# ITBE-Lab/ma

Measured on AMD Instinct MI355X. Metric: aligned reads/sec (whole node), 150bp & 10kb synthetic vs GRCh38, higher is better.
Workload: dtype u8/int8 (2-bit BWT ranks, int8 DP differences, int16/32 scores); 1 GPU; 20000000 x 150 bp reads (0.50% sub, 0.00% ins, 0.00% del), default preset, 1000000 reads/step per GPU vs GRCh38-like synthetic genome (24 contigs, 3088269832 nt, planted repeats)

## Files before the change

ma_amd/csrc/launch_seed.h:

```cpp
static SeedParams seed_params( const ma_params& P )
{
    SeedParams S;
    S.technique = (u32)P.seeding_technique;
    S.min_seed_len = (u32)P.min_seed_len;
    S.min_amb = (u32)P.min_ambiguity;
    S.max_amb = (u32)P.max_ambiguity;
    S.min_seed_size_drop = (u32)P.min_seed_size_drop;
    S.disable_heuristics = (u32)P.disable_heuristics;
    S.rel_min_seed_size_amount = P.rel_min_seed_size_amount;
    S.genome_size_disable = P.genome_size_disable;
    S.window_begin = S.window_end = nullptr;
    S.smem_compact = 0;
    S.smem_merge = 0;
    return S;
}
static void seed_window( SeedParams& S, const ma_batch* b, bool on )
{
    const u64 bytes = b->n_bases + ( b->reads_external ? 0 : 64 );
    if( const char* e = getenv( "MA_SEED_WINDOW" ) )
        on = on && atoi( e ) != 0;
    if( on && bytes >= 16 )
    {
        S.window_begin = b->d_reads;
        S.window_end = b->d_reads + bytes;
    }
}

static int seed_mems( ma_batch* b )
{
    const u64 n = b->n_reads, nb = b->n_bases;
    if( b->segOff.reserve( ( n + 1 ) * 8 ) || b->segCnt.reserve( ( n + 1 ) * 4 ) || b->memsCnt.reserve( ( nb + 2 ) * 8 ) ||
        b->memsOff.reserve( ( nb + 2 ) * 8 ) )
        return 1;
    MemsArgs A;
    A.X = b->idx->v;
    A.P = seed_params( b->P );
    A.reads = b->d_reads;
    A.roff = b->d_roff;
    A.n_reads = (u32)n;
    A.n_bases = nb;
    A.cnt = b->memsCnt.as<u64>( );
    A.off = b->memsOff.as<u64>( );
    A.pool = nullptr;
    A.pool_read = nullptr;
    A.ctr = b->ctr.as<unsigned long long>( );
    EvTimer t( b, 0 );
    u64 total = 0;
    if( nb )
    {
        hipLaunchKernelGGL( k_mems<false>, dim3( (unsigned)( ( nb + 255 ) / 256 ) ), dim3( 256 ), 0, b->stream, A );
        MA_HIP( hipMemsetAsync( (char*)b->memsCnt.p + nb * 8, 0, 8, b->stream ) );
        if( scan_exclusive<u64>( b, b->memsCnt.as<u64>( ), b->memsOff.as<u64>( ), nb + 1 ) )
            return 1;
        MA_HIP( hipMemcpyAsync( &total, (char*)b->memsOff.p + nb * 8, 8, hipMemcpyDeviceToHost, b->stream ) );
        if( batch_wait( b ) )
        return 1;
    }
    else
        MA_HIP( hipMemsetAsync( b->memsOff.p, 0, 16, b->stream ) );
    b->segPoolCap = std::max<u64>( total + 1024, b->segPoolCap );
    if( b->segPool.reserve( b->segPoolCap * sizeof( ma_segment ) ) || b->segRead.reserve( b->segPoolCap * 4 ) )
        return 1;
    A.pool = b->segPool.as<ma_segment>( );
    A.pool_read = b->segRead.as<u32>( );
    if( nb && total )
        hipLaunchKernelGGL( k_mems<true>, dim3( (unsigned)( ( nb + 255 ) / 256 ) ), dim3( 256 ), 0, b->stream, A );
    hipLaunchKernelGGL( k_mems_finish, dim3( (unsigned)( ( n + 255 ) / 256 ) ), dim3( 256 ), 0, b->stream, A.X, A.P, b->d_roff, (u32)n,
                        b->memsOff.as<u64>( ), b->segPool.as<ma_segment>( ), b->segOff.as<u64>( ), b->segCnt.as<u32>( ) );
    const unsigned long long used = total;
    MA_HIP( hipMemcpyAsync( b->ctr.as<unsigned long long>( ) + CTR_SEG_USED, &used, 8, hipMemcpyHostToDevice, b->stream ) );
    if( batch_wait( b ) )
        return 1;
    MA_HIP( hipGetLastError( ) );
    return 0;
}

static u64 seg_pool_heuristic( u64 n_bases, u64 n_reads )
{
    return std::max<u64>( n_bases / 16 + 16 * n_reads, 1024 );
}

static int seed_tasks( ma_batch* b )
{
    const u64 n = b->n_reads, nb = b->n_bases;
    int levels = 2;
    for( u32 q = b->max_qlen; q > 1; q >>= 1 )
        levels++;
    if( levels >= MA_TASK_KEY_BITS / 2 )
        return 2;
    const bool smem = b->P.seeding_technique == 1;
    const u64 taskCap = nb / 16 + 2 * n + 1024;
    b->segPoolCap = std::max( ( smem ? 4 : 1 ) * seg_pool_heuristic( nb, n ), b->segPoolMin );
    u32 segCapT = 96, smemCapT = 384;
    if( const char* e = getenv( "MA_SEED_TASK_CAPS" ) )
    {
        int a = 0, c = 0;
        if( sscanf( e, "%d,%d", &a, &c ) == 2 && a > 0 && c > 0 )
            segCapT = (u32)a, smemCapT = (u32)( ( c + 1 ) & ~1 );
    }
    const u32 smem_compact = smem && b->max_qlen < ( 1u << MA_SMEM_QZ_BITS ) && b->idx->v.n < ( 1ull << 35 ) && !( getenv( "MA_SMEM_COMPACT" ) && atoi( getenv( "MA_SMEM_COMPACT" ) ) == 0 ) ? 1 : 0;
    const u64 smemEntry = smem_compact ? 16 : sizeof( ma_segment );
    unsigned blocksT = smem ? 1024 : 2048;
    if( const char* e = getenv( "MA_SEED_TASK_BLOCKS" ) )
        blocksT = (unsigned)std::max( 64, std::min( 4096, atoi( e ) ) );
    const u64 lanesT = (u64)blocksT * 256;
    if( smem && ( b->taskStage.reserve( lanesT * segCapT * sizeof( ma_segment ) ) || b->smemA.reserve( lanesT * smemCapT * smemEntry ) ||
                  b->smemB.reserve( lanesT * smemCapT * smemEntry ) ) )
        return 1;
    if( b->segOff.reserve( ( n + 1 ) * 8 ) || b->segCnt.reserve( ( n + 1 ) * 4 ) || b->taskA.reserve( taskCap * sizeof( SeedTask ) ) ||
        b->taskB.reserve( taskCap * sizeof( SeedTask ) ) || b->taskCnt.reserve( 64 * 8 ) ||
        b->segPool.reserve( b->segPoolCap * sizeof( ma_segment ) ) || b->segRead.reserve( b->segPoolCap * 4 ) ||
        b->stage.reserve( b->segPoolCap * sizeof( ma_segment ) ) || b->taskKey.reserve( b->segPoolCap * 8 ) ||
        b->taskKey2.reserve( b->segPoolCap * 8 ) || b->taskPerm.reserve( b->segPoolCap * 4 ) || b->taskPerm2.reserve( b->segPoolCap * 4 ) )
        return 1;
    unsigned long long* cnt = b->taskCnt.as<unsigned long long>( );
    MA_HIP( hipMemsetAsync( cnt, 0, 64 * 8, b->stream ) );
    TaskKernelArgs A;
    A.X = b->idx->v;
    A.P = seed_params( b->P );
    seed_window( A.P, b, true );
    A.slow_batch = 4;
    if( const char* e = getenv( "MA_SEED_SLOW_BATCH" ) )
        A.slow_batch = (u32)std::max( 1, atoi( e ) );
    A.reads = b->d_reads;
    A.roff = b->d_roff;
    A.task_cap = taskCap;
    A.pool = b->stage.as<ma_segment>( );
    A.pool_key = b->taskKey.as<u64>( );
    A.pool_cap = b->segPoolCap;
    A.ctr = b->ctr.as<unsigned long long>( );
    A.stage = smem ? b->taskStage.as<ma_segment>( ) : nullptr;
    A.seg_cap = segCapT;
    A.smem_a = smem ? b->smemA.as<ma_segment>( ) : nullptr;
    A.smem_b = smem ? b->smemB.as<ma_segment>( ) : nullptr;
    A.smem_cap = smemCapT;
    if( smem )
    {
        A.P.smem_compact = smem_compact;
        A.P.smem_merge = A.P.min_amb == 0 ? 1 : 0;
        if( const char* e = getenv( "MA_SMEM_MERGE" ) )
            A.P.smem_merge = A.P.smem_merge && atoi( e ) != 0 ? 1 : 0;
        A.X.kmer_k = 0;
        A.slow_batch = 8;
        if( const char* e = getenv( "MA_SEED_SLOW_BATCH" ) )
            A.slow_batch = (u32)std::max( 1, atoi( e ) );
    }
    {
        EvTimer t( b, 0 );
        hipLaunchKernelGGL( k_task_roots, dim3( (unsigned)( ( n + 255 ) / 256 ) ), dim3( 256 ), 0, b->stream, b->d_roff, (u32)n,
                            b->taskA.as<SeedTask>( ), cnt );
        for( int lv = 0; lv < levels; lv++ )
        {
            A.in = ( lv & 1 ) ? b->taskB.as<SeedTask>( ) : b->taskA.as<SeedTask>( );
            A.out = ( lv & 1 ) ? b->taskA.as<SeedTask>( ) : b->taskB.as<SeedTask>( );
            A.nIn = cnt + lv;
            A.nOut = cnt + lv + 1;
            MA_HIP( hipMemsetAsync( A.ctr + CTR_NEXT_READ, 0, 8, b->stream ) );
            if( smem )
                hipLaunchKernelGGL( k_seed_tasks_smem, dim3( blocksT ), dim3( 256 ), 0, b->stream, A );
            else
                hipLaunchKernelGGL( k_seed_tasks, dim3( blocksT ), dim3( 256 ), 0, b->stream, A );
        }
    }
    MA_HIP( hipGetLastError( ) );
    if( read_ctr( b ) )
        return 1;
    const u32 err = (u32)b->hctr[ CTR_ERR ];
    const u64 ns = b->hctr[ CTR_SEG_USED ];
    if( ( err & ( MA_ERR_STACK_OVERFLOW | MA_ERR_SMEM_OVERFLOW ) ) )
    {
        MA_HIP( hipMemsetAsync( b->ctr.p, 0, CTR_COUNT * 8, b->stream ) );
        return 2;
    }
    if( ( err & MA_ERR_SEG_OVERFLOW ) || ns > b->segPoolCap )
    {
        b->segPoolMin = ns + 1024;
        MA_HIP( hipMemsetAsync( b->ctr.p, 0, CTR_COUNT * 8, b->stream ) );
        return seed_tasks( b );
    }
    MA_HIP( hipMemsetAsync( b->segCnt.p, 0, ( n + 1 ) * 4, b->stream ) );
    if( ns )
    {
        hipLaunchKernelGGL( k_iota32, dim3( (unsigned)( ( ns + 255 ) / 256 ) ), dim3( 256 ), 0, b->stream, b->taskPerm.as<u32>( ), ns );
        size_t tb = 0;
        MA_HIP( hipcub::DeviceRadixSort::SortPairs( nullptr, tb, b->taskKey.as<u64>( ), b->taskKey2.as<u64>( ), b->taskPerm.as<u32>( ),
                                                    b->taskPerm2.as<u32>( ), (int)ns, 0, 64, b->stream ) );
        if( b->cubTmp.reserve( tb + 256 ) )
            return 1;
        MA_HIP( hipcub::DeviceRadixSort::SortPairs( b->cubTmp.p, tb, b->taskKey.as<u64>( ), b->taskKey2.as<u64>( ), b->taskPerm.as<u32>( ),
                                                    b->taskPerm2.as<u32>( ), (int)ns, 0, 64, b->stream ) );
        const dim3 grid( (unsigned)( ( ns + 255 ) / 256 ) ), block( 256 );
        hipLaunchKernelGGL( k_task_permute, grid, block, 0, b->stream, b->stage.as<ma_segment>( ), b->taskKey2.as<u64>( ),
                            b->taskPerm2.as<u32>( ), ns, b->segPool.as<ma_segment>( ), b->segRead.as<u32>( ) );
        hipLaunchKernelGGL( k_task_ranges, grid, block, 0, b->stream, b->segRead.as<u32>( ), ns, b->segOff.as<u64>( ), b->segCnt.as<u32>( ) );
    }
    hipLaunchKernelGGL( k_task_finish, dim3( (unsigned)( ( n + 255 ) / 256 ) ), dim3( 256 ), 0, b->stream, b->idx->v, seed_params( b->P ),
                        b->d_roff, (u32)n, b->segPool.as<ma_segment>( ), b->segOff.as<u64>( ), b->segCnt.as<u32>( ) );
    MA_HIP( hipGetLastError( ) );
    return 0;
}

static int seed_run( ma_batch* b )
{
    const u64 n = b->n_reads;
    MA_HIP( hipMemsetAsync( b->ctr.p, 0, CTR_COUNT * 8, b->stream ) );
    if( n == 0 )
        return 0;
    if( b->P.seeding_technique == 2 )
        return seed_mems( b );
    {
        bool tasks = b->P.seeding_technique <= 1 && b->max_qlen > 240 && n < 65536;
        if( const char* e = getenv( "MA_SEED_TASKS" ) )
            tasks = b->P.seeding_technique <= 1 && atoi( e ) != 0;
        if( tasks )
        {
            const int rc = seed_tasks( b );
            if( rc != 2 )
                return rc;
        }
    }
    const bool smem = b->P.seeding_technique == 1;
    const u32 worst_cap = ( smem ? 6 : 2 ) * b->max_qlen + 8;
    const u32 smem_cap = smem ? ( ( b->max_qlen + 3 ) & ~1u ) : 0;
    b->segPoolCap = seg_pool_heuristic( b->n_bases, n );
    if( smem )
        b->segPoolCap *= 4;
    b->segPoolCap = std::max( b->segPoolCap, b->segPoolMin );
    if( const char* e = getenv( "MA_SEG_POOL_CAP" ) )
        if( b->segPoolMin == 0 )
            b->segPoolCap = (u64)std::max( 1, atoi( e ) );
    size_t freeB = 0, totalB = 0;
    MA_HIP( hipMemGetInfo( &freeB, &totalB ) );
    const u64 have = b->stage.cap + b->smemA.cap + b->smemB.cap;
    const u64 budget = std::max<u64>( 8ull << 30, ( (u64)freeB + have ) / 3 );
    u64 want = std::min<u64>( 256ull * 2048, ( n + 255 ) / 256 * 256 );
    if( const char* e = getenv( "MA_SEED_LANES" ) )
        want = std::min<u64>( want, std::max<u64>( 256, (u64)atoll( e ) / 256 * 256 ) );
    u32 smem_compact = smem && b->max_qlen < ( 1u << MA_SMEM_QZ_BITS ) && b->idx->v.n < ( 1ull << 35 ) ? 1 : 0;
    if( const char* e = getenv( "MA_SMEM_COMPACT" ) )
        smem_compact = smem_compact && atoi( e ) != 0 ? 1 : 0;
    const u64 smem_entry = smem_compact ? 16 : sizeof( ma_segment );
    u32 seg_cap = worst_cap;
    if( want * ( (u64)worst_cap * sizeof( ma_segment ) + 2ull * smem_cap * smem_entry ) > budget )
        seg_cap = std::min<u32>( worst_cap, ( smem ? 3 : 1 ) * ( b->max_qlen / 4 ) + 64 );
    if( const char* e = getenv( "MA_SEED_STAGE_CAP" ) )
        seg_cap = std::min<u32>( worst_cap, (u32)std::max( 1, atoi( e ) ) );
    for( int attempt = 0; attempt < 3; attempt++ )
    {
        const u64 lane_bytes = (u64)seg_cap * sizeof( ma_segment ) + 2ull * smem_cap * smem_entry;
        const u64 lanes = std::min<u64>( want, std::max<u64>( 256, ( budget / lane_bytes ) / 256 * 256 ) );
        if( b->stage.reserve( lanes * seg_cap * sizeof( ma_segment ) ) ||
            ( smem && ( b->smemA.reserve( lanes * smem_cap * smem_entry ) || b->smemB.reserve( lanes * smem_cap * smem_entry ) ) ) ||
            b->segPool.reserve( b->segPoolCap * sizeof( ma_segment ) ) || b->segRead.reserve( b->segPoolCap * 4 ) ||
            b->segOff.reserve( n * 8 ) || b->segCnt.reserve( n * 4 ) || b->seedStack.reserve( lanes * 2 * MA_SEED_STACK * 4 ) )
            return 1;
        SeedKernelArgs A;
        A.X = b->idx->v;
        A.P = seed_params( b->P );
        A.reads = b->d_reads;
        A.roff = b->d_roff;
        A.n_reads = (u32)n;
        A.stage = b->stage.as<ma_segment>( );
        A.seg_cap = seg_cap;
        A.smem_a = smem ? b->smemA.as<ma_segment>( ) : nullptr;
        A.smem_b = smem ? b->smemB.as<ma_segment>( ) : nullptr;
        A.smem_cap = smem_cap;
        A.stack = b->seedStack.as<u32>( );
        A.pool = b->segPool.as<ma_segment>( );
        A.pool_read = b->segRead.as<u32>( );
        A.pool_cap = b->segPoolCap;
        A.seg_off = b->segOff.as<u64>( );
        A.seg_cnt = b->segCnt.as<u32>( );
        A.ctr = b->ctr.as<unsigned long long>( );
        {
            EvTimer t( b, 0 );
            const u32 qb = (u32)( ( b->max_qlen + 7 ) / 8 * 8 + 4 );
            A.q_lds = qb * 256 <= 64 * 1024 ? qb : 0;
            seed_window( A.P, b, A.q_lds == 0 );
            A.P.smem_compact = smem_compact;
            A.P.smem_merge = smem && A.P.min_amb == 0 ? 1 : 0;
            if( const char* e = getenv( "MA_SMEM_MERGE" ) )
                A.P.smem_merge = A.P.smem_merge && atoi( e ) != 0 ? 1 : 0;
            A.slow_batch = A.P.technique == 0 ? ( A.q_lds ? 4 : 16 ) : 8;
            if( const char* e = getenv( "MA_SEED_SLOW_BATCH" ) )
                A.slow_batch = (u32)std::max( 1, atoi( e ) );
            bool text = !smem && A.q_lds && A.P.min_amb == 0;
            if( const char* e = getenv( "MA_SEED_TEXT" ) )
                text = text && atoi( e ) != 0;
            if( text )
            {
                b->st.markSegments( true );
                hipLaunchKernelGGL( ( k_seed<false, true> ), dim3( (unsigned)( lanes / 256 ) ), dim3( 256 ), A.q_lds * 256, b->stream, A );
            }
            else if( A.q_lds )
                hipLaunchKernelGGL( smem ? k_seed<true> : k_seed<false>, dim3( (unsigned)( lanes / 256 ) ), dim3( 256 ), A.q_lds * 256, b->stream, A );
            else
            {
                if( const char* e = getenv( "MA_SEED_LONG_JUMP" ) )
                    if( atoi( e ) == 0 )
                        A.X.kmer_k = 0;
                hipLaunchKernelGGL( smem ? k_seed_long<true> : k_seed_long<false>, dim3( (unsigned)( lanes / 256 ) ), dim3( 256 ), 0, b->stream, A );
            }
        }
        MA_HIP( hipGetLastError( ) );
        if( read_ctr( b ) )
            return 1;
        if( !( (u32)b->hctr[ CTR_ERR ] & MA_ERR_SEG_OVERFLOW ) )
            break;
        bool retry = false;
        if( b->hctr[ CTR_SEG_USED ] > b->segPoolCap )
        {
            b->segPoolMin = b->segPoolCap = b->hctr[ CTR_SEG_USED ] + 1024;
            retry = true;
        }
        if( seg_cap < worst_cap )
        {
            seg_cap = worst_cap;
            retry = true;
        }
        if( !retry || attempt == 2 )
            break;
        MA_HIP( hipMemsetAsync( b->ctr.p, 0, CTR_COUNT * 8, b->stream ) );
    }
    return 0;
}

int ma_seed_batch( ma_batch* b )
{
    if( !b || !b->d_roff )
        return fail( "ma_seed_batch: no reads set" );
    MA_BIND_DEVICE( b->device );
    b->st.drop( ma_state::SEEDED );
    if( seed_run( b ) )
        return 1;
    b->st.finish( ma_state::SEEDED );
    return 0;
}
```

ma_amd/csrc/stage_seed.h:

```cpp
struct SeedKernelArgs
{
    IndexView X;
    SeedParams P;
    const uint8_t* reads;
    const u64* roff;
    u32 n_reads;
    ma_segment* stage;
    u32 seg_cap;
    ma_segment* smem_a;
    ma_segment* smem_b;
    u32 smem_cap;
    u32* stack;
    u32 q_lds;
    u32 slow_batch;
    ma_segment* pool;
    u32* pool_read;
    u64 pool_cap;
    u64* seg_off;
    u32* seg_cnt;
    unsigned long long* ctr;
};

#if defined( MA_KSW_PROF )
static __device__ unsigned long long g_seed_prof[ 8 ];
#endif
#define MA_SMEM_LDS_HEADS_TASK 6
template <bool LONG, bool SM, bool TXT = false, bool MS = !SM> __device__ __forceinline__ void seed_kernel_body( const SeedKernelArgs& A )
{
    const u32 lane = blockIdx.x * blockDim.x + threadIdx.x;
    SeedScratch S;
    S.stage = A.stage + (u64)lane * A.seg_cap;
    S.seg_cap = A.seg_cap;
    const u64 smemWords = (u64)A.smem_cap * ( A.P.smem_compact ? 2u : 5u );
    S.smem_a = A.smem_a ? (ma_segment*)( (u64*)A.smem_a + (u64)lane * smemWords ) : nullptr;
    S.smem_b = A.smem_b ? (ma_segment*)( (u64*)A.smem_b + (u64)lane * smemWords ) : nullptr;
    S.smem_cap = A.smem_cap;
    S.stack = A.stack + (u64)lane * ( 2 * MA_SEED_STACK );
    S.drop_div = A.P.min_seed_size_drop;
    SeedLane L;
    L.phase = PH_DONE;
    u32 read = 0xffffffffu;
    u64 steps = 0, blocks = 0;
    const u32 wl = threadIdx.x & 63;
#if defined( MA_KSW_PROF )
    unsigned long long pf[ 7 ] = { 0, 0, 0, 0, 0, 0, 0 };
#endif
    extern __shared__ __attribute__( ( aligned( 16 ) ) ) uint8_t q_lds[];
    uint8_t* myq = q_lds + (size_t)threadIdx.x * A.q_lds;
    bool alive = true;
    while( true )
    {
        const bool done = alive && L.phase == PH_DONE;
        const unsigned long long dm = __ballot( done );
#if defined( MA_KSW_PROF )
        const unsigned long long tA = clock64( );
#endif
        if( dm && ( __popcll( dm ) >= 8 || dm == __ballot( alive ) ) )
        {
            const bool flush = done && read != 0xffffffffu;
            const u32 n = flush ? seed_finish( L, A.P, S, A.X ) : 0u;
            u32 inc = n;
            for( int d = 1; d < 64; d <<= 1 )
            {
                const u32 o = (u32)__shfl_up( (int)inc, d, 64 );
                if( wl >= (u32)d )
                    inc += o;
            }
            const u32 total = (u32)__shfl( (int)inc, 63, 64 );
            unsigned long long base = 0, rb = 0;
            if( wl == 0 )
            {
                rb = atomicAdd( &A.ctr[ CTR_NEXT_READ ], (unsigned long long)__popcll( dm ) );
                base = atomicAdd( &A.ctr[ CTR_SEG_USED ], (unsigned long long)total );
            }
            base = ( (u64)(u32)__shfl( (int)( base >> 32 ), 0, 64 ) << 32 ) | (u32)__shfl( (int)(u32)base, 0, 64 );
            rb = ( (u64)(u32)__shfl( (int)( rb >> 32 ), 0, 64 ) << 32 ) | (u32)__shfl( (int)(u32)rb, 0, 64 );
            if( flush )
            {
                const u64 off = base + inc - n;
                if( off + n <= A.pool_cap )
                {
                    const ma_segment* __restrict__ src = S.stage;
                    ma_segment* __restrict__ dst = A.pool + off;
                    u32* __restrict__ dr = A.pool_read + off;
#pragma unroll 4
                    for( u32 k = 0; k < n; k++ )
                    {
                        dst[ k ] = src[ k ];
                        dr[ k ] = read;
                    }
                }
                else
                    L.err |= MA_ERR_SEG_OVERFLOW;
                A.seg_off[ read ] = off;
                A.seg_cnt[ read ] = off + n <= A.pool_cap ? n : 0;
                if( L.err )
                    atomicOr( (unsigned long long*)&A.ctr[ CTR_ERR ], (unsigned long long)L.err );
                steps += L.steps;
                blocks += L.blocks;
            }
            if( done )
            {
                const u64 mine = rb + (u64)__popcll( dm & ( ( 1ull << wl ) - 1 ) );
                if( mine >= A.n_reads )
                    alive = false;
                else
                {
                    read = (u32)mine;
                    const uint8_t* src = A.reads + A.roff[ read ];
                    const u32 ql = (u32)( A.roff[ read + 1 ] - A.roff[ read ] );
                    if( !LONG )
                    {
                        u32 k = 0;
                        for( ; k + 16 <= ql; k += 16 )
                        {
                            uint4 v;
                            __builtin_memcpy( &v, src + k, 16 );
                            u32* d = (u32*)( myq + k );
                            d[ 0 ] = v.x, d[ 1 ] = v.y, d[ 2 ] = v.z, d[ 3 ] = v.w;
                        }
                        for( ; k < ql; k++ )
                            myq[ k ] = src[ k ];
                        src = myq;
                    }
                    seed_begin_read( L, src, ql );
                }
            }
        }
        if( __ballot( alive ) == 0 )
            break;
#if defined( MA_KSW_PROF )
        const unsigned long long tB = clock64( );
#endif
        u32 c = 0;
        const bool act = alive && L.phase != PH_DONE;
        bool ext = act && seed_try<LONG, SM, MS>( L, A.P, c, &S );
        {
            const unsigned long long sm = __ballot( act && !ext );
#if defined( MA_KSW_PROF )
            const unsigned long long tB1 = clock64( );
            if( sm && ( (u32)__popcll( sm ) >= A.slow_batch || __ballot( ext ) == 0 ) )
                pf[ 5 ] += 1ull << 32, pf[ 0 ] -= tB1;
#endif
            if( sm && ( (u32)__popcll( sm ) >= A.slow_batch || __ballot( ext ) == 0 ) )
                if( act && !ext )
                    ext = seed_prepare<LONG, true, SM, MS, TXT>( L, A.P, S, A.X, c );
#if defined( MA_KSW_PROF )
            if( sm && ( (u32)__popcll( sm ) >= A.slow_batch || __ballot( ext ) == 0 ) )
                pf[ 0 ] += clock64( );
#endif
        }
#if defined( MA_KSW_PROF )
        const unsigned long long tC = clock64( );
        pf[ 4 ] += __popcll( __ballot( ext ) );
#endif
        if( ext )
        {
            if( LONG )
                seed_prefetch<LONG>( L, A.P );
            seed_step<TXT, SM, MS, !LONG>( L, A.P, S, A.X, c );
        }
#if defined( MA_KSW_PROF )
        const unsigned long long tD = clock64( );
        pf[ 6 ] += tB - tA;
        pf[ 1 ] += tC - tB;
        pf[ 2 ] += tD - tC;
        pf[ 3 ] += 1;
        pf[ 5 ] += dm ? 1 : 0;
#endif
    }
#if defined( MA_KSW_PROF )
    if( wl == 0 )
        for( int i = 0; i < 6; i++ )
            atomicAdd( &g_seed_prof[ i ], pf[ i ] );
#endif
    atomicAdd( &A.ctr[ CTR_STEPS ], (unsigned long long)steps );
    atomicAdd( &A.ctr[ CTR_BLOCKS ], (unsigned long long)blocks );
}
template <bool SM, bool TXT = false> __global__ void __launch_bounds__( 256 ) k_seed( SeedKernelArgs A )
{
    seed_kernel_body<false, SM, TXT>( A );
}
template <bool SM> __global__ void __launch_bounds__( 256 ) __attribute__( ( amdgpu_waves_per_eu( 4 ) ) ) k_seed_long( SeedKernelArgs A )
{
    seed_kernel_body<true, SM>( A );
}

__global__ void k_seg_materialise( IndexView X, const uint8_t* reads, const u64* roff, const u32* pool_read, ma_segment* pool, u64 n )
{
    const u64 i = (u64)blockIdx.x * blockDim.x + threadIdx.x;
    if( i >= n )
        return;
    ma_segment s = pool[ i ];
    if( s.sa_start >= 0 )
        return;
    seed_materialise( X, reads + roff[ pool_read[ i ] ], s );
    pool[ i ] = s;
}

__device__ __forceinline__ u64 wave_sum_u64( u64 v );
struct MemsArgs
{
    IndexView X;
    SeedParams P;
    const uint8_t* reads;
    const u64* roff;
    u32 n_reads;
    u64 n_bases;
    u64* cnt;
    const u64* off;
    ma_segment* pool;
    u32* pool_read;
    unsigned long long* ctr;
};
struct MemsCount
{
    u64 n = 0;
    MA_HD void emit( u32, u32, i64, i64 )
    {
        n++;
    }
};
struct MemsFill
{
    ma_segment* out;
    u32* out_read;
    u32 read;
    u64 n = 0;
    MA_HD void emit( u32 qs, u32 qsz, i64 sa, i64 san )
    {
        ma_segment s;
        s.q_start = qs, s.q_size = qsz, s.sa_start = sa, s.sa_start_rc = -1, s.sa_size = san;
        out[ n ] = s;
        out_read[ n ] = read;
        n++;
    }
};
template <bool FILL> __global__ void __launch_bounds__( 256 ) k_mems( MemsArgs A )
{
    const u64 t = (u64)blockIdx.x * blockDim.x + threadIdx.x;
    u64 steps = 0, blocks = 0;
    if( t < A.n_bases )
    {
        const u64 b = A.roff[ 0 ] + t;
        u32 lo = 0, hi = A.n_reads;
        while( hi - lo > 1 )
        {
            const u32 mid = ( lo + hi ) / 2;
            if( A.roff[ mid ] <= b )
                lo = mid;
            else
                hi = mid;
        }
        const u64 r0 = A.roff[ lo ];
        const u32 qlen = (u32)( A.roff[ lo + 1 ] - r0 ), i = (u32)( b - r0 );
        if( FILL )
        {
            MemsFill sink{ A.pool + A.off[ t ], A.pool_read + A.off[ t ], lo };
            if( A.off[ t + 1 ] > A.off[ t ] )
                mems_from( A.X, A.P, A.reads + r0, qlen, i, sink, steps, blocks );
        }
        else
        {
            MemsCount sink;
            mems_from( A.X, A.P, A.reads + r0, qlen, i, sink, steps, blocks );
            A.cnt[ t ] = sink.n;
        }
    }
    if( !FILL )
    {
        steps = wave_sum_u64( steps );
        blocks = wave_sum_u64( blocks );
        if( ( threadIdx.x & 63 ) == 0 && steps )
        {
            atomicAdd( &A.ctr[ CTR_STEPS ], (unsigned long long)steps );
            atomicAdd( &A.ctr[ CTR_BLOCKS ], (unsigned long long)blocks );
        }
    }
}
__global__ void k_mems_finish( IndexView X, SeedParams P, const u64* roff, u32 n_reads, const u64* off, ma_segment* pool, u64* seg_off,
                               u32* seg_cnt )
{
    const u32 r = blockIdx.x * blockDim.x + threadIdx.x;
    if( r >= n_reads )
        return;
    const u64 b = off[ roff[ r ] - roff[ 0 ] ], e = off[ roff[ r + 1 ] - roff[ 0 ] ];
    u32 n = (u32)( e - b );
    if( !P.disable_heuristics && P.min_seed_size_drop != 0 )
    {
        u64 sum = 0;
        for( u64 k = b; k < e; k++ )
            sum += (u64)pool[ k ].q_size / (u64)P.min_seed_size_drop;
        if( (double)sum < P.rel_min_seed_size_amount * (double)( roff[ r + 1 ] - roff[ r ] ) && P.genome_size_disable < X.n )
        {
            for( u64 k = b; k < e; k++ )
                pool[ k ].q_size = 0, pool[ k ].sa_size = 0;
            n = 0;
        }
    }
    seg_off[ r ] = b;
    seg_cnt[ r ] = n;
}

struct SeedTask
{
    u32 read, aS, aN, depth;
    u64 key;
};
#define MA_TASK_KEY_BITS 40
struct TaskKernelArgs
{
    IndexView X;
    SeedParams P;
    const uint8_t* reads;
    const u64* roff;
    const SeedTask* in;
    const unsigned long long* nIn;
    SeedTask* out;
    unsigned long long* nOut;
    u64 task_cap;
    ma_segment* pool;
    u64* pool_key;
    u64 pool_cap;
    unsigned long long* ctr;
    u32 slow_batch;
    ma_segment* stage;
    u32 seg_cap;
    ma_segment* smem_a;
    ma_segment* smem_b;
    u32 smem_cap;
};
__global__ void k_task_roots( const u64* roff, u32 n_reads, SeedTask* out, unsigned long long* nOut )
{
    const u32 r = blockIdx.x * blockDim.x + threadIdx.x;
    if( r == 0 )
        *nOut = n_reads;
    if( r >= n_reads )
        return;
    SeedTask t;
    t.read = r, t.aS = 0, t.aN = (u32)( roff[ r + 1 ] - roff[ r ] ), t.depth = 0, t.key = 0;
    out[ r ] = t;
}
template <bool SM> __device__ __forceinline__ void seed_tasks_body( const TaskKernelArgs& A )
{
    constexpr bool MS = !SM;
    const u32 wl = threadIdx.x & 63;
    if( A.ctr[ CTR_ERR ] & MA_ERR_STACK_OVERFLOW )
        return;
    const u64 nIn = *A.nIn < A.task_cap ? *A.nIn : A.task_cap;
    SeedLane L;
    L.phase = PH_DONE;
    L.err = 0;
    ma_segment mine[ 2 ];
    SeedScratch S;
    S.stage = mine;
    S.seg_cap = 2;
    S.smem_a = S.smem_b = nullptr;
    S.smem_cap = 0;
    if( SM )
    {
        const u64 lane = (u64)blockIdx.x * blockDim.x + threadIdx.x;
        const u64 smemWords = (u64)A.smem_cap * ( A.P.smem_compact ? 2u : 5u );
        S.stage = A.stage + lane * A.seg_cap;
        S.seg_cap = A.seg_cap;
        S.smem_a = (ma_segment*)( (u64*)A.smem_a + lane * smemWords );
        S.smem_b = (ma_segment*)( (u64*)A.smem_b + lane * smemWords );
        S.smem_cap = A.smem_cap;
    }
    __shared__ ulonglong2 sHeads[ SM ? 2 * MA_SMEM_LDS_HEADS_TASK * 256 : 1 ];
    if( SM && A.P.smem_compact )
    {
        S.lds = (u64*)sHeads + 2 * threadIdx.x;
        S.lds_n = A.smem_cap < MA_SMEM_LDS_HEADS_TASK ? A.smem_cap : MA_SMEM_LDS_HEADS_TASK;
        S.lds_stride = 256;
    }
    S.stack = nullptr;
    S.drop_div = 0;
    SeedTask T;
    T.read = 0xffffffffu;
    bool alive = true;
    u64 steps = 0, blocks = 0;
    u64 qCur = 0, qEnd = 0;
    while( true )
    {
        const bool done = alive && L.phase == PH_DONE;
        const unsigned long long dm = __ballot( done ), am = __ballot( alive );
        if( dm && ( __popcll( dm ) >= 8 || dm == am ) )
        {
            const bool flush = done && T.read != 0xffffffffu;
            if( SM && flush && ( L.err & ( MA_ERR_SEG_OVERFLOW | MA_ERR_SMEM_OVERFLOW ) ) )
                L.err = ( L.err & ~(u32)MA_ERR_SEG_OVERFLOW ) | MA_ERR_SMEM_OVERFLOW;
            const u32 ns = flush ? ( L.nseg < S.seg_cap ? L.nseg : S.seg_cap ) : 0;
            const u32 nc = flush ? ( L.childN[ 0 ] ? 1 : 0 ) + ( L.childN[ 1 ] ? 1 : 0 ) : 0;
            u32 incS = ns, incC = nc;
            for( int d = 1; d < 64; d <<= 1 )
            {
                const u32 o = (u32)__shfl_up( (int)incS, d, 64 ), o2 = (u32)__shfl_up( (int)incC, d, 64 );
                if( wl >= (u32)d )
                    incS += o, incC += o2;
            }
            const u32 totS = (u32)__shfl( (int)incS, 63, 64 ), totC = (u32)__shfl( (int)incC, 63, 64 );
            unsigned long long baseS = 0, baseC = 0;
            if( wl == 0 )
            {
                if( totS )
                    baseS = atomicAdd( &A.ctr[ CTR_SEG_USED ], (unsigned long long)totS );
                if( totC )
                    baseC = atomicAdd( A.nOut, (unsigned long long)totC );
            }
            baseS = ( (u64)(u32)__shfl( (int)( baseS >> 32 ), 0, 64 ) << 32 ) | (u32)__shfl( (int)(u32)baseS, 0, 64 );
            baseC = ( (u64)(u32)__shfl( (int)( baseC >> 32 ), 0, 64 ) << 32 ) | (u32)__shfl( (int)(u32)baseC, 0, 64 );
            if( flush )
            {
                const u64 so = baseS + incS - ns, co = baseC + incC - nc;
                if( so + ns <= A.pool_cap )
                    for( u32 k = 0; k < ns; k++ )
                    {
                        A.pool[ so + k ] = SM ? S.stage[ k ] : mine[ k ];
                        A.pool_key[ so + k ] = ( (u64)T.read << MA_TASK_KEY_BITS ) | T.key;
                    }
                else
                    L.err |= MA_ERR_SEG_OVERFLOW;
                if( co + nc <= A.task_cap && T.depth + 1 < MA_TASK_KEY_BITS / 2 )
                {
                    u32 w = 0;
                    for( int side = 0; side < 2; side++ )
                        if( L.childN[ side ] )
                        {
                            SeedTask c;
                            c.read = T.read, c.aS = L.childS[ side ], c.aN = L.childN[ side ], c.depth = T.depth + 1;
                            c.key = T.key | ( (u64)( side + 1 ) << ( MA_TASK_KEY_BITS - 2 * ( T.depth + 1 ) ) );
                            A.out[ co + w++ ] = c;
                        }
                }
                else if( nc )
                    L.err |= MA_ERR_STACK_OVERFLOW;
                if( L.err )
                    atomicOr( (unsigned long long*)&A.ctr[ CTR_ERR ], (unsigned long long)L.err );
                steps += L.steps;
                blocks += L.blocks;
                T.read = 0xffffffffu;
            }
            if( qCur == qEnd )
            {
                unsigned long long base = 0;
                if( wl == 0 )
                    base = atomicAdd( &A.ctr[ CTR_NEXT_READ ], 256ull );
                base = ( (u64)(u32)__shfl( (int)( base >> 32 ), 0, 64 ) << 32 ) | (u32)__shfl( (int)(u32)base, 0, 64 );
                qCur = base < nIn ? base : nIn;
                qEnd = base + 256 < nIn ? base + 256 : nIn;
            }
            const u64 avail = qEnd - qCur;
            const u64 rank = (u64)__popcll( dm & ( ( 1ull << wl ) - 1 ) );
            if( done )
            {
                if( rank < avail )
                {
                    T = A.in[ qCur + rank ];
                    const u64 r0 = A.roff[ T.read ];
                    seed_begin_area( L, A.reads + r0, (u32)( A.roff[ T.read + 1 ] - r0 ), T.aS, T.aN );
                }
                else if( qEnd == nIn )
                    alive = false;
            }
            const u64 want = (u64)__popcll( dm );
            qCur += want < avail ? want : avail;
        }
        if( __ballot( alive ) == 0 )
            break;
        u32 c = 0;
        const bool act = alive && L.phase != PH_DONE;
        bool ext = act && seed_try<true, SM, MS>( L, A.P, c, SM ? &S : nullptr );
        {
            const unsigned long long sm = __ballot( act && !ext );
            if( sm && ( (u32)__popcll( sm ) >= A.slow_batch || __ballot( ext ) == 0 ) )
                if( act && !ext )
                    ext = seed_prepare<true, true, SM, MS>( L, A.P, S, A.X, c );
        }
        if( ext )
        {
            i64 ok[ 3 ];
            u32 nb;
            seed_prefetch<true>( L, A.P );
            extend_backward( A.X, L.ik, c, ok, nb );
            L.steps++;
            L.blocks += nb;
            seed_apply<SM, MS>( L, A.P, S, ok );
        }
    }
    steps = wave_sum_u64( steps );
    blocks = wave_sum_u64( blocks );
    if( wl == 0 && steps )
    {
        atomicAdd( &A.ctr[ CTR_STEPS ], (unsigned long long)steps );
        atomicAdd( &A.ctr[ CTR_BLOCKS ], (unsigned long long)blocks );
    }
}
__global__ void __launch_bounds__( 256 ) k_seed_tasks( TaskKernelArgs A )
{
    seed_tasks_body<false>( A );
}
#if !defined( MA_TASKS_SMEM_WAVES )
#define MA_TASKS_SMEM_WAVES 3
#endif
__global__ void __launch_bounds__( 256 ) __attribute__( ( amdgpu_waves_per_eu( MA_TASKS_SMEM_WAVES ) ) ) k_seed_tasks_smem( TaskKernelArgs A )
{
    seed_tasks_body<true>( A );
}
__global__ void k_task_permute( const ma_segment* in, const u64* sorted_key, const u32* perm, u64 n, ma_segment* out, u32* out_read )
{
    const u64 i = (u64)blockIdx.x * blockDim.x + threadIdx.x;
    if( i >= n )
        return;
    out[ i ] = in[ perm[ i ] ];
    out_read[ i ] = (u32)( sorted_key[ i ] >> MA_TASK_KEY_BITS );
}
__global__ void k_iota32( u32* p, u64 n )
{
    const u64 i = (u64)blockIdx.x * blockDim.x + threadIdx.x;
    if( i < n )
        p[ i ] = (u32)i;
}
__global__ void k_task_ranges( const u32* seg_read, u64 n, u64* seg_off, u32* seg_cnt )
{
    const u64 i = (u64)blockIdx.x * blockDim.x + threadIdx.x;
    if( i >= n )
        return;
    const u32 r = seg_read[ i ];
    if( i == 0 || seg_read[ i - 1 ] != r )
        seg_off[ r ] = i;
    if( i + 1 == n || seg_read[ i + 1 ] != r )
        seg_cnt[ r ] = (u32)( i + 1 );
}
__global__ void k_task_finish( IndexView X, SeedParams P, const u64* roff, u32 n_reads, ma_segment* pool, u64* seg_off, u32* seg_cnt )
{
    const u32 r = blockIdx.x * blockDim.x + threadIdx.x;
    if( r >= n_reads )
        return;
    if( seg_cnt[ r ] == 0 )
    {
        seg_off[ r ] = 0;
        return;
    }
    const u64 b = seg_off[ r ], e = seg_cnt[ r ];
    u32 n = (u32)( e - b );
    if( !P.disable_heuristics && P.min_seed_size_drop != 0 )
    {
        u64 sum = 0;
        for( u64 k = b; k < e; k++ )
            sum += (u64)pool[ k ].q_size / (u64)P.min_seed_size_drop;
        if( (double)sum < P.rel_min_seed_size_amount * (double)( roff[ r + 1 ] - roff[ r ] ) && P.genome_size_disable < X.n )
        {
            for( u64 k = b; k < e; k++ )
                pool[ k ].q_size = 0, pool[ k ].sa_size = 0;
            n = 0;
        }
    }
    seg_cnt[ r ] = n;
}
```

Measured before the change: 42.24 million aligned reads/s.

## Add per-wave read queue and cooperative coalesced query copy into LDS

```diff
diff --git a/ma_amd/csrc/launch_seed.h b/ma_amd/csrc/launch_seed.h
--- a/ma_amd/csrc/launch_seed.h
+++ b/ma_amd/csrc/launch_seed.h
@@ -284,6 +284,16 @@
             A.slow_batch = A.P.technique == 0 ? ( A.q_lds ? 4 : 16 ) : 8;
             if( const char* e = getenv( "MA_SEED_SLOW_BATCH" ) )
                 A.slow_batch = (u32)std::max( 1, atoi( e ) );
+            A.refill = 1;
+            if( const char* e = getenv( "MA_SEED_REFILL" ) )
+                A.refill = atoi( e ) != 0 ? 1 : 0;
+            A.refill_at = 8;
+            if( const char* e = getenv( "MA_SEED_REFILL_AT" ) )
+                A.refill_at = (u32)std::max( 1, std::min( 64, atoi( e ) ) );
+            A.slice = 8;
+            if( const char* e = getenv( "MA_SEED_SLICE" ) )
+                A.slice = (u32)std::max( 0, std::min( 4096, atoi( e ) ) );
+            A.slice = A.q_lds && n > lanes ? (u32)std::min<u64>( A.slice, ( n - lanes ) / ( lanes / 64 ) / 2 ) : 0;
             bool text = !smem && A.q_lds && A.P.min_amb == 0;
             if( const char* e = getenv( "MA_SEED_TEXT" ) )
                 text = text && atoi( e ) != 0;
diff --git a/ma_amd/csrc/seed_refill.h b/ma_amd/csrc/seed_refill.h
--- /dev/null
+++ b/ma_amd/csrc/seed_refill.h
@@ -0,0 +1,105 @@
+#pragma once
+#include "ma_common.h"
+
+namespace ma
+{
+struct RefillQueue
+{
+    u32 cur = 0, end = 0;
+    u32 newB = 0, newE = 0;
+    bool dry = false;
+};
+MA_HD u32 refill_queue_ask( const RefillQueue& q, u32 nd, u32 slice )
+{
+    return nd > q.end - q.cur && !q.dry ? nd - ( q.end - q.cur ) + slice : 0u;
+}
+MA_HD void refill_queue_answer( RefillQueue& q, u64 before, u32 ask, u32 n_reads )
+{
+    q.newB = (u32)( before < n_reads ? before : n_reads );
+    q.newE = (u32)( before + ask < n_reads ? before + ask : n_reads );
+    q.dry = before + ask >= n_reads;
+}
+MA_HD u32 refill_queue_read( const RefillQueue& q, u32 rank )
+{
+    const u32 avail = q.end - q.cur;
+    if( rank < avail )
+        return q.cur + rank;
+    return rank - avail < q.newE - q.newB ? q.newB + ( rank - avail ) : 0xffffffffu;
+}
+MA_HD void refill_queue_served( RefillQueue& q, u32 nd, bool asked )
+{
+    const u32 avail = q.end - q.cur;
+    if( nd <= avail )
+        q.cur += nd;
+    else if( asked )
+        q.cur = q.newB + mmin( nd - avail, q.newE - q.newB ), q.end = q.newE;
+    else
+        q.cur = q.end;
+    q.newB = q.newE = 0;
+}
+
+MA_HD u32 refill_chunks( u32 ql )
+{
+    return ( ql + 15u ) >> 4;
+}
+MA_HD u32 refill_div_factor( u32 ch )
+{
+    return ( 65536u + ch - 1u ) / ch;
+}
+MA_HD u32 refill_div( u32 c, u32 factor )
+{
+    return ( c * factor ) >> 16;
+}
+#define MA_REFILL_MAX_QLEN 255u
+MA_HD u32 refill_pack( u32 ql, u32 owner )
+{
+    return ( ql << 6 ) | owner;
+}
+MA_HD u32 refill_qlen( u32 pk )
+{
+    return pk >> 6;
+}
+MA_HD u32 refill_owner( u32 pk )
+{
+    return pk & 63u;
+}
+MA_HD u32 refill_chunk_words( u32 off, u32 ql )
+{
+    return off >= ql ? 0u : mmin( 4u, ( ql - off + 3u ) >> 2 );
+}
+MA_HD bool refill_chunk_whole( const uint8_t* p, const uint8_t* end )
+{
+    return (size_t)( end - p ) >= 16;
+}
+MA_HD void refill_chunk_load_whole( const uint8_t* p, u32& w0, u32& w1, u32& w2, u32& w3 )
+{
+    u32 w[ 4 ];
+    __builtin_memcpy( w, p, 16 );
+    w0 = w[ 0 ], w1 = w[ 1 ], w2 = w[ 2 ], w3 = w[ 3 ];
+}
+MA_HD void refill_chunk_load( const uint8_t* p, const uint8_t* end, u32& w0, u32& w1, u32& w2, u32& w3 )
+{
+    if( refill_chunk_whole( p, end ) )
+    {
+        refill_chunk_load_whole( p, w0, w1, w2, w3 );
+        return;
+    }
+    const u32 have = (u32)( end - p );
+    w0 = w1 = w2 = w3 = 0;
+#if defined( __HIPCC__ )
+#pragma unroll
+#endif
+    for( u32 k = 0; k < 16; k++ )
+    {
+        const u32 b = k < have ? (u32)p[ k ] << ( 8u * ( k & 3u ) ) : 0u;
+        if( k < 4 )
+            w0 |= b;
+        else if( k < 8 )
+            w1 |= b;
+        else if( k < 12 )
+            w2 |= b;
+        else
+            w3 |= b;
+    }
+}
+}
diff --git a/ma_amd/csrc/stage_seed.h b/ma_amd/csrc/stage_seed.h
--- a/ma_amd/csrc/stage_seed.h
+++ b/ma_amd/csrc/stage_seed.h
@@ -1,3 +1,4 @@
+#include "seed_refill.h"
 struct SeedKernelArgs
 {
     IndexView X;
@@ -5,6 +6,9 @@
     const uint8_t* reads;
     const u64* roff;
     u32 n_reads;
+    u32 refill;
+    u32 refill_at;
+    u32 slice;
     ma_segment* stage;
     u32 seg_cap;
     ma_segment* smem_a;
@@ -48,6 +52,8 @@
     extern __shared__ __attribute__( ( aligned( 16 ) ) ) uint8_t q_lds[];
     uint8_t* myq = q_lds + (size_t)threadIdx.x * A.q_lds;
     bool alive = true;
+    RefillQueue Q;
+    constexpr bool COOP = !LONG && !SM;
     while( true )
     {
         const bool done = alive && L.phase == PH_DONE;
@@ -55,7 +61,7 @@
 #if defined( MA_KSW_PROF )
         const unsigned long long tA = clock64( );
 #endif
-        if( dm && ( __popcll( dm ) >= 8 || dm == __ballot( alive ) ) )
+        if( dm && ( (u32)__popcll( dm ) >= A.refill_at || dm == __ballot( alive ) ) )
         {
             const bool flush = done && read != 0xffffffffu;
             const u32 n = flush ? seed_finish( L, A.P, S, A.X ) : 0u;
@@ -68,13 +74,30 @@
             }
             const u32 total = (u32)__shfl( (int)inc, 63, 64 );
             unsigned long long base = 0, rb = 0;
+            const u32 nd = (u32)__popcll( dm ), ask = refill_queue_ask( Q, nd, A.slice );
             if( wl == 0 )
             {
-                rb = atomicAdd( &A.ctr[ CTR_NEXT_READ ], (unsigned long long)__popcll( dm ) );
-                base = atomicAdd( &A.ctr[ CTR_SEG_USED ], (unsigned long long)total );
+                if( ask )
+                    rb = atomicAdd( &A.ctr[ CTR_NEXT_READ ], (unsigned long long)ask );
+                if( total )
+                    base = atomicAdd( &A.ctr[ CTR_SEG_USED ], (unsigned long long)total );
             }
             base = ( (u64)(u32)__shfl( (int)( base >> 32 ), 0, 64 ) << 32 ) | (u32)__shfl( (int)(u32)base, 0, 64 );
             rb = ( (u64)(u32)__shfl( (int)( rb >> 32 ), 0, 64 ) << 32 ) | (u32)__shfl( (int)(u32)rb, 0, 64 );
+            if( ask )
+                refill_queue_answer( Q, rb, ask, A.n_reads );
+            u32 nread = 0xffffffffu, ql = 0;
+            u64 ro = 0;
+            const u64 roEnd = COOP && A.refill ? A.roff[ A.n_reads ] : 0;
+            if( done )
+            {
+                nread = refill_queue_read( Q, (u32)__popcll( dm & ( ( 1ull << wl ) - 1 ) ) );
+                if( nread != 0xffffffffu )
+                {
+                    ro = A.roff[ nread ];
+                    ql = (u32)( A.roff[ nread + 1 ] - ro );
+                }
+            }
             if( flush )
             {
                 const u64 off = base + inc - n;
@@ -99,32 +122,103 @@
                 steps += L.steps;
                 blocks += L.blocks;
             }
+            refill_queue_served( Q, nd, ask != 0 );
+            const bool fresh = done && nread != 0xffffffffu;
             if( done )
             {
-                const u64 mine = rb + (u64)__popcll( dm & ( ( 1ull << wl ) - 1 ) );
-                if( mine >= A.n_reads )
+                if( fresh )
+                    read = nread;
+                else
                     alive = false;
-                else
+            }
+            if( COOP && A.refill )
+            {
+                const unsigned long long fm = __ballot( fresh );
+                const u32 chn = fresh ? refill_chunks( ql ) : 0u;
+                u32 CH = 0;
+#pragma unroll
+                for( int bit = 4; bit >= 0; bit-- )
+                    if( __ballot( chn >= ( CH | ( 1u << bit ) ) ) )
+                        CH |= 1u << bit;
+                if( CH )
                 {
-                    read = (u32)mine;
-                    const uint8_t* src = A.reads + A.roff[ read ];
-                    const u32 ql = (u32)( A.roff[ read + 1 ] - A.roff[ read ] );
-                    if( !LONG )
+                    const u32 nf = (u32)__popcll( fm ), rank = (u32)__popcll( fm & ( ( 1ull << wl ) - 1 ) );
+                    const int to = (int)( ( fresh ? rank : nf + wl - rank ) * 4u );
+                    const u32 tbl = (u32)__builtin_amdgcn_ds_permute( to, (int)refill_pack( ql, wl ) );
+                    const u32 tblLo = (u32)__builtin_amdgcn_ds_permute( to, (int)(u32)ro ), tblHi = (u32)__builtin_amdgcn_ds_permute( to, (int)( ro >> 32 ) );
+                    const u32 fac = refill_div_factor( CH ), nch = nf * CH;
+                    const uint8_t* srcEnd = A.reads + roEnd;
+                    uint8_t* wq = q_lds + (size_t)( threadIdx.x & ~63u ) * A.q_lds;
+                    for( u32 cb = 0; cb < nch; cb += 128 )
                     {
-                        u32 k = 0;
-                        for( ; k + 16 <= ql; k += 16 )
+                        const u32 c0 = cb + wl, c1 = c0 + 64;
+                        const u32 d0 = refill_div( c0, fac ), d1 = refill_div( c1, fac );
+                        const u32 p0 = (u32)__shfl( (int)tbl, (int)( d0 & 63u ), 64 ), p1 = (u32)__shfl( (int)tbl, (int)( d1 & 63u ), 64 );
+                        const u64 r0 = ( (u64)(u32)__shfl( (int)tblHi, (int)( d0 & 63u ), 64 ) << 32 ) | (u32)__shfl( (int)tblLo, (int)( d0 & 63u ), 64 );
+                        const u64 r1 = ( (u64)(u32)__shfl( (int)tblHi, (int)( d1 & 63u ), 64 ) << 32 ) | (u32)__shfl( (int)tblLo, (int)( d1 & 63u ), 64 );
+                        const u32 o0 = 16u * ( c0 - d0 * CH ), o1 = 16u * ( c1 - d1 * CH );
+                        const u32 n0 = c0 < nch ? refill_chunk_words( o0, refill_qlen( p0 ) ) : 0u;
+                        const u32 n1 = c1 < nch ? refill_chunk_words( o1, refill_qlen( p1 ) ) : 0u;
+                        u32 a0 = 0, a1 = 0, a2 = 0, a3 = 0, b0 = 0, b1 = 0, b2 = 0, b3 = 0;
+                        const uint8_t *s0 = A.reads + r0 + o0, *s1 = A.reads + r1 + o1;
+                        if( __ballot( ( n0 && !refill_chunk_whole( s0, srcEnd ) ) || ( n1 && !refill_chunk_whole( s1, srcEnd ) ) ) == 0 )
                         {
-                            uint4 v;
-                            __builtin_memcpy( &v, src + k, 16 );
-                            u32* d = (u32*)( myq + k );
-                            d[ 0 ] = v.x, d[ 1 ] = v.y, d[ 2 ] = v.z, d[ 3 ] = v.w;
+                            if( n0 )
+                                refill_chunk_load_whole( s0, a0, a1, a2, a3 );
+                            if( n1 )
+                                refill_chunk_load_whole( s1, b0, b1, b2, b3 );
                         }
-                        for( ; k < ql; k++ )
-                            myq[ k ] = src[ k ];
-                        src = myq;
+                        else
+                        {
+                            if( n0 )
+                                refill_chunk_load( s0, srcEnd, a0, a1, a2, a3 );
+                            if( n1 )
+                                refill_chunk_load( s1, srcEnd, b0, b1, b2, b3 );
+                        }
+                        u32* da = (u32*)( wq + (size_t)refill_owner( p0 ) * A.q_lds + o0 );
+                        u32* db = (u32*)( wq + (size_t)refill_owner( p1 ) * A.q_lds + o1 );
+                        if( n0 > 0 )
+                            da[ 0 ] = a0;
+                        if( n0 > 1 )
+                            da[ 1 ] = a1;
+                        if( n0 > 2 )
+                            da[ 2 ] = a2;
+                        if( n0 > 3 )
+                            da[ 3 ] = a3;
+                        if( n1 > 0 )
+                            db[ 0 ] = b0;
+                        if( n1 > 1 )
+                            db[ 1 ] = b1;
+                        if( n1 > 2 )
+                            db[ 2 ] = b2;
+                        if( n1 > 3 )
+                            db[ 3 ] = b3;
                     }
-                    seed_begin_read( L, src, ql );
+                    __builtin_amdgcn_fence( __ATOMIC_RELEASE, "wavefront" );
+                    __builtin_amdgcn_wave_barrier( );
+                    __builtin_amdgcn_fence( __ATOMIC_ACQUIRE, "wavefront" );
                 }
+                if( fresh )
+                    seed_begin_read( L, myq, ql );
+            }
+            else if( fresh )
+            {
+                const uint8_t* src = A.reads + ro;
+                if( !LONG )
+                {
+                    u32 k = 0;
+                    for( ; k + 16 <= ql; k += 16 )
+                    {
+                        uint4 v;
+                        __builtin_memcpy( &v, src + k, 16 );
+                        u32* d = (u32*)( myq + k );
+                        d[ 0 ] = v.x, d[ 1 ] = v.y, d[ 2 ] = v.z, d[ 3 ] = v.w;
+                    }
+                    for( ; k < ql; k++ )
+                        myq[ k ] = src[ k ];
+                    src = myq;
+                }
+                seed_begin_read( L, src, ql );
             }
         }
         if( __ballot( alive ) == 0 )
```

After: 42.88 million aligned reads/s (median of 6 runs). No clear change (+1.5%).
